# junyanz/interactive-deep-colorization

Measured on NVIDIA H100. Metric: net_forward images/sec @256x256, higher is better.
Workload: dtype f16x2-split operands, f32 accumulate (ab within 1e-3 of the f32 reference)

## Files before the change

### interactive_deep_colorization_b200/csrc/idc_api.cu

```cuda
#include <math.h>
#include <stdarg.h>
#include <stdio.h>
#include <string.h>

#include <algorithm>

#include "idc_internal.h"

using namespace idc;

struct idc_ctx : public idc::Ctx {};

namespace {

int fail(Ctx* c, int code, const char* fmt, ...) {
  char buf[512];
  va_list ap;
  va_start(ap, fmt);
  vsnprintf(buf, sizeof(buf), fmt, ap);
  va_end(ap);
  if (c) c->err = buf;
  return code;
}

// ... 545 lines not shown
                                    (size_t)nk * 2 * HW * sizeof(float), cudaMemcpyDeviceToHost, c->s_out));
      }
    } else {
      const int cap = (forked && c->click_mode && c->d_clickout) ? side_branch_cap(c) : 0;
      CUDA_TRY(c, umma_run_op(c, op, n, op.fuse_out_head ? out_ab : nullptr, (float)c->opt.tanh_scale, st, 0, cap));
    }
    mark();
  }
  const bool fused = !c->simt && !(c->flags & IDC_FLAG_KEEP_CONV10);
  if (!fused) CUDA_TRY(c, launch_out_head(c, n, out_ab, st));
  if (out_dist && !forked) {
    CUDA_TRY(c, launch_softmax529(c, n, out_dist, st));
    CUDA_TRY(c, click_tail(c, n, st));
    pdl_break(c);
  }
  if (out_rgb) {
    CUDA_TRY(c, launch_lab2rgb(c, n, c->H, c->W, L, 50.0f, out_ab, out_rgb, st, out_abq));
    c->launch_count++;
  }
  if (forked) {
    CUDA_TRY(c, cudaStreamWaitEvent(st, c->ev_join, 0));
    pdl_break(c);
  }
  mark();
  pdl_break(c);
  c->last_n = n;
  return IDC_OK;
}

int check_forward_args(Ctx* c, int n, int h, int w, const void* L, const void* ab, const void* mask, const void* glob,
                       const void* out_ab, const void* out_dist, bool resident_l_ok = false, bool hints_ok = false) {
  if (!c->weights_ready) return fail(c, IDC_ERR_STATE, "idc_forward before idc_finalize_weights");
  if (n < 1 || n > c->max_n) return fail(c, IDC_ERR_ARG, "n=%d outside [1,%d]", n, c->max_n);
  if (h != c->H || w != c->W) return fail(c, IDC_ERR_ARG, "geometry %dx%d != ctx geometry %dx%d", h, w, c->H, c->W);
  const bool hint_mode = hints_ok && !ab && !mask;
  if ((!L && !resident_l_ok) || ((!ab || !mask) && !hint_mode) || !out_ab)
    return fail(c, IDC_ERR_ARG, "null L/ab/mask/out_ab");
  if (out_dist && !c->dist) return fail(c, IDC_ERR_ARG, "out_dist requires IDC_FLAG_DIST");
  if (glob && !c->glob) return fail(c, IDC_ERR_ARG, "glob requires IDC_FLAG_GLOBAL_HINTS");
  return IDC_OK;
}

}

extern "C" {

const char* idc_version(void) { return "idc_b200 0.2 sm_90a (wgmma split-fp16 + fp32 simt engines)"; }

int idc_create(int device, int max_n, int h, int w, unsigned flags, idc_ctx** out) {
  if (!out) return IDC_ERR_ARG;
  *out = nullptr;
  if (max_n < 1 || h < 8 || w < 8 || (h % 8) || (w % 8)) return IDC_ERR_ARG;
  int ndev = 0;
  if (cudaGetDeviceCount(&ndev) != cudaSuccess || device < 0 || device >= ndev) return IDC_ERR_CUDA;
  cudaDeviceProp prop;
  if (cudaGetDeviceProperties(&prop, device) != cudaSuccess) return IDC_ERR_CUDA;
  if (prop.major != 9 || prop.minor != 0) return IDC_ERR_UNSUPPORTED;
  if (cudaSetDevice(device) != cudaSuccess) return IDC_ERR_CUDA;
  idc_ctx* c = new idc_ctx();
  c->dev = device; c->max_n = max_n; c->H = h; c->W = w; c->flags = flags;
  c->simt = flags & IDC_FLAG_ENGINE_SIMT;
  c->fast = (flags & IDC_FLAG_FAST_FP16) && !c->simt;
  c->dist = flags & IDC_FLAG_DIST;
  c->glob = flags & IDC_FLAG_GLOBAL_HINTS;
  c->caffe313 = flags & IDC_FLAG_CAFFE313;
  build_plan(c);
  int rc = alloc_workspace(c);
  if (rc != IDC_OK) {
    fprintf(stderr, "idc_create: %s\n", c->err.c_str());
    idc_destroy(c);
    return rc;
  }
  cudaStreamCreateWithFlags(&c->own_stream, cudaStreamNonBlocking);
  *out = c;
  return IDC_OK;
}

int idc_set_option(idc_ctx* c, const char* name, int value) {
  if (!c || !name) return IDC_ERR_ARG;
  struct { const char* n; int* v; } tab[] = {
      {"halo", &c->opt.halo}, {"pairs", &c->opt.pairs}, {"mt", &c->opt.mt},
      {"chunk_kb", &c->opt.chunk_kb}, {"split_k", &c->opt.split_k}, {"host_pipe", &c->opt.host_pipe},
      {"pdl", &c->opt.pdl}, {"tanh_scale", &c->opt.tanh_scale}, {"side_dist", &c->opt.side_dist},
      {"conv1_1_umma", &c->opt.conv1_1_umma}};
  for (auto& t : tab)
    if (!strcmp(t.n, name)) {
      *t.v = value;
      if (c->weights_ready && strcmp(name, "host_pipe") && strcmp(name, "tanh_scale") && strcmp(name, "side_dist") && strcmp(name, "conv1_1_umma")) {
        CUDA_TRY(c, cudaSetDevice(c->dev));
        CUDA_TRY(c, cudaDeviceSynchronize());
        int rc = plan_engines(c);
        if (rc != IDC_OK) return rc;
      }
      if (c->graph_exec) { cudaGraphExecDestroy(c->graph_exec); c->graph_exec = nullptr; }
      return IDC_OK;
    }
  return fail(c, IDC_ERR_KEY, "unknown option '%s'", name);
}

int idc_load_tensor(idc_ctx* c, const char* key, const void* data, int dtype, int ndim, const int64_t* dims) {
  if (!c || !key || !data || ndim < 0 || ndim > 8 || (ndim && !dims)) return fail(c, IDC_ERR_ARG, "bad load_tensor args");
  HostTensor t;
  size_t count = 1;
  for (int i = 0; i < ndim; ++i) {
    if (dims[i] < 0) return fail(c, IDC_ERR_ARG, "negative dim");
    t.dims.push_back(dims[i]);
    count *= (size_t)dims[i];
  }
  t.data.resize(count);
  switch (dtype) {
    case IDC_F32: memcpy(t.data.data(), data, count * sizeof(float)); break;
    case IDC_F64: for (size_t i = 0; i < count; ++i) t.data[i] = (float)((const double*)data)[i]; break;
    case IDC_I64: for (size_t i = 0; i < count; ++i) t.data[i] = (float)((const int64_t*)data)[i]; break;
    default: return fail(c, IDC_ERR_ARG, "unknown dtype %d", dtype);
  }
  c->raw[key] = std::move(t);
  c->weights_ready = false;
  return IDC_OK;
}

int idc_reserve_weights(idc_ctx* c) {
  if (!c) return IDC_ERR_ARG;
  CUDA_TRY(c, cudaSetDevice(c->dev));
  if (!c->arena) {
    c->arena_bytes = layout_arena(c, nullptr);
    CUDA_TRY(c, cudaMalloc(&c->arena, c->arena_bytes));
    layout_arena(c, c->arena);
  }
  return IDC_OK;
}

int idc_finalize_weights(idc_ctx* c) {
  if (!c) return IDC_ERR_ARG;
  int rc = idc_reserve_weights(c);
  if (rc != IDC_OK) return rc;
  std::vector<char> host(c->arena_bytes, 0);
  rc = pack_weights(c, host.data());
  if (rc != IDC_OK) return rc;
  if (c->caffe313) {
    const HostTensor* pts = find(c, "caffe.pts_in_hull");
    if (!check_dims(pts, {313, 2})) return fail(c, IDC_ERR_KEY, "missing/bad caffe.pts_in_hull [313,2]");
    CUDA_TRY(c, cudaMemcpy(c->pts313, pts->data.data(), sizeof(float) * 626, cudaMemcpyHostToDevice));
  }
  CUDA_TRY(c, cudaMemcpy(c->arena, host.data(), c->arena_bytes, cudaMemcpyHostToDevice));
  return idc_adopt_weights(c);
}

int idc_adopt_weights(idc_ctx* c) {
  if (!c || !c->arena) return fail(c, IDC_ERR_STATE, "no arena");
  CUDA_TRY(c, cudaSetDevice(c->dev));
  int rc = plan_engines(c);
  if (rc != IDC_OK) return rc;
  CUDA_TRY(c, cudaMemcpy(c->h_w11.w, c->w11, sizeof(c->h_w11.w), cudaMemcpyDeviceToHost));
  CUDA_TRY(c, cudaMemcpy(c->h_w11.b, c->b11, sizeof(c->h_w11.b), cudaMemcpyDeviceToHost));
  if (!c->simt) CUDA_TRY(c, conv1_1_umma_pack(c));
  c->raw.clear();
  c->weights_ready = true;
  if (c->graph_exec) { cudaGraphExecDestroy(c->graph_exec); c->graph_exec = nullptr; }
  return IDC_OK;
}

int idc_weights_arena(idc_ctx* c, void** dev_ptr, size_t* bytes) {
  if (!c || !dev_ptr || !bytes) return IDC_ERR_ARG;
  if (!c->arena) return fail(c, IDC_ERR_STATE, "arena not allocated");
  *dev_ptr = c->arena; *bytes = c->arena_bytes;
  return IDC_OK;
}
// ... 703 lines not shown
```

### interactive_deep_colorization_b200/csrc/idc_internal.h

```cpp
#pragma once
#include <cuda.h>
#include <cuda_fp16.h>
#include <cuda_runtime.h>
#include <stdint.h>

#include <map>
#include <string>
#include <vector>

#include "../../include/idc_b200.h"

namespace idc {

constexpr int kMaxTaps = 34;
constexpr int kMaxSrc = 6;
constexpr int kMaxCls = 4;

enum Act { ACT_NONE = 0, ACT_RELU = 1, ACT_LEAKY02 = 2 };

constexpr int kActScaleLog2 = 6;
constexpr float kActScale = 64.0f;
constexpr float kActInvScale = 1.0f / 64.0f;

struct Tap {
  int src;
  int ky, kx;
  int ty, tx;
};

struct ActBuf {
  std::string name;
  int H = 0, W = 0, C = 0;
  void* p0 = nullptr;
  void* p1 = nullptr;
};

struct Epilogue {
  float* bias = nullptr;
  float* scale = nullptr;
  float* shift = nullptr;
  int act = ACT_NONE;
  bool has_bn = false;
  bool gadd = false;
};

struct SrcDesc {
  int buf = -1;
  int s = 1;
  int cin = 0;
};

enum OpKind { OP_CONV = 0, OP_UP = 1, OP_CLASS = 2, OP_HYPER = 3 };

struct ConvOp {
  std::string name;
  int kind = OP_CONV;
  std::string wkey[kMaxSrc];
  bool src_deconv[kMaxSrc] = {false, false, false, false, false, false};
  int src_k[kMaxSrc] = {3, 3, 3, 3, 3, 3};
  std::string bnkey;
  int nsrc = 1;
  SrcDesc src[kMaxSrc];
  int ncls = 1;
  int ntaps = 0;
  Tap taps[kMaxCls][kMaxTaps];
  int Hl = 0, Wl = 0;
  int out_buf = -1;
  int os = 1;
  int cout = 0, cout_pad = 0;
  int K = 0;
  Epilogue epi;
  bool fuse_out_head = false;
  bool out_f32 = false;
  float* out_f32_ptr = nullptr;
  float* w_simt = nullptr;
  __half* w_hi = nullptr;
  __half* w_lo = nullptr;
  int bn_tile = 0, hbox = 0, wbox = 0;
  void* umma_plan = nullptr;
  double flops_per_image = 0;
};

struct Conv11Weights {
  float w[36 * 64];
  float b[64];
};

struct Options {
  int halo = 1;
  int pairs = 0;
  int mt = -1;
  int chunk_kb = -1;
  int split_k = -1;
  int host_pipe = 1;
  int pdl = 1;
  int conv1_1_umma = 1;
  int side_dist = 1;
  int tanh_scale = 110;
};

struct HostTensor {
  std::vector<float> data;
  std::vector<int64_t> dims;
};

struct Ctx {
  int dev = 0;
  int max_n = 0, H = 0, W = 0;
  unsigned flags = 0;
  Options opt;
  bool simt = false, fast = false, dist = false, glob = false;
  std::map<std::string, HostTensor> raw;
  std::vector<ActBuf> bufs;
  std::map<std::string, int> buf_index;
  std::vector<ConvOp> ops;
  char* arena = nullptr;
  size_t arena_bytes = 0;
  bool weights_ready = false;
  float* w11 = nullptr;
  float* b11 = nullptr;
  Conv11Weights h_w11;
  uint8_t* w11_umma = nullptr;
  float* wout = nullptr;
  float* bout = nullptr;
  float* gw[4] = {nullptr, nullptr, nullptr, nullptr};
  float* gb[4] = {nullptr, nullptr, nullptr, nullptr};
  float* gscale[4] = {nullptr, nullptr, nullptr, nullptr};
  float* gshift[4] = {nullptr, nullptr, nullptr, nullptr};
  float* gvec = nullptr;
  float* gtmp = nullptr;
  float* logits = nullptr;
  float* logits313 = nullptr;
  bool caffe313 = false;
  float* pts313 = nullptr;
  float* splitk_ws = nullptr; size_t splitk_ws_floats = 0;
  int* splitk_counters = nullptr; int splitk_max_tiles = 0;
  bool dbg_graph_timing = false;
  cudaEvent_t dbg_ev[2] = {nullptr, nullptr};
  float dbg_graph_ms = 0.f;
  int* d_err = nullptr;
  int* h_err = nullptr;
  float* h_in = nullptr;  float* d_in = nullptr;   size_t in_floats = 0;
  float* h_out = nullptr; float* d_out = nullptr;  size_t out_floats = 0;
  uint8_t* h_rgb = nullptr; uint8_t* d_rgb = nullptr;
  char* h_small = nullptr; char* d_small = nullptr;
  double* h_abq = nullptr; double* d_abq = nullptr;
  cudaStream_t own_stream = nullptr;
  cudaStream_t s_in = nullptr, s_out = nullptr;
  cudaStream_t s_side = nullptr;
  cudaEvent_t ev_fork = nullptr, ev_join = nullptr;
  cudaStream_t s_click = nullptr;
  cudaEvent_t ev_click[2] = {nullptr, nullptr};
  int image_n = 0;
  char* h_hints = nullptr; char* d_hints = nullptr;
  int graph_captures = 0;
  cudaEvent_t ev_in[8] = {}, ev_out[8] = {};
  cudaGraphExec_t graph_exec = nullptr;
  const void* graph_ptrs[8] = {nullptr};
  float graph_maskcent = 0.f;
  int launch_count = 0;
  int graph_launches = 0;
  bool chain = false;
  bool gadd_active = false;
  int last_n = 0;
  double* d_reccs = nullptr;
  bool dist_resident = false;
  int dist_valid_n = 0;
  bool click_mode = false;
  int* h_click = nullptr; int* d_click = nullptr;
  char* d_clickout = nullptr; char* h_clickout = nullptr;
  bool click_served = false;
  bool profiling = false;
  std::vector<std::vector<cudaEvent_t>> prof_runs;
  std::vector<cudaEvent_t> prof_pool;
  std::string err;
};
// ... 67 lines not shown
```

### interactive_deep_colorization_b200/csrc/idc_umma.cu

```cuda
#include <stdio.h>
#include <stdlib.h>

#include "idc_internal.h"

namespace idc {

constexpr int kBM = 128;
constexpr int kBK = 64;
constexpr int kThreads = 384;
constexpr int kProdRegs = 40;
constexpr int kMathRegs = 232;
constexpr int kMathThreads = 256;

struct UmmaParams {
  const CUtensorMap* amaps;
  const int4* kblk;
  int nkb, ncls;
  int chunk_kb;
  int split_k;
  float* ws;
  int* counters;
  int n_img, tiles_y, tiles_x, n_tiles_n, total_tiles;
  int hbox, wbox, wshift;
  int Hl, Wl, cout_pad;
  const float* bias;
  const float* scale;
  const float* shift;
  const float* gadd;
  int gadd_ld;
  float gadd_mult;
  int act;
  __half* out_hi;
  __half* out_lo;
  int Hout, Wout, Cout, os;
  float* out_f32;
  int out_ld;
  const float* wout;
  const float* bout;
  float* out_ab;
  float out_mult;
  int* err;
  int n_amaps;
  int max_ctas;
  int img0;
};

__device__ __forceinline__ uint32_t smem_u32(const void* p) { return (uint32_t)__cvta_generic_to_shared(p); }

__device__ __forceinline__ void mbar_init(uint32_t bar, uint32_t count) {
  asm volatile("mbarrier.init.shared::cta.b64 [%0], %1;" ::"r"(bar), "r"(count));
}
__device__ __forceinline__ void mbar_expect_tx(uint32_t bar, uint32_t bytes) {
  asm volatile("mbarrier.arrive.expect_tx.shared::cta.b64 _, [%0], %1;" ::"r"(bar), "r"(bytes) : "memory");
}
__device__ __forceinline__ void mbar_arrive(uint32_t bar) {
  asm volatile("mbarrier.arrive.shared::cta.b64 _, [%0];" ::"r"(bar) : "memory");
}
__device__ __forceinline__ uint32_t mbar_try_wait(uint32_t bar, uint32_t parity) {
  uint32_t ok;
  asm volatile(
      "{\n\t.reg .pred p;\n\t"
      "mbarrier.try_wait.parity.shared::cta.b64 p, [%1], %2;\n\t"
      "selp.u32 %0, 1, 0, p;\n\t}"
      : "=r"(ok)
      : "r"(bar), "r"(parity)
      : "memory");
  return ok;
}
__device__ __noinline__ void mbar_timeout(int* err, int code) {
  if (err) {
    atomicExch(err, code);
    __threadfence_system();
  }
  __trap();
}
__device__ __forceinline__ void mbar_wait(uint32_t bar, uint32_t parity, int* err, int code) {
  if (mbar_try_wait(bar, parity)) return;
  const long long t0 = clock64();
  while (!mbar_try_wait(bar, parity)) {
    if (clock64() - t0 > 6000000000LL) mbar_timeout(err, code);
  }
}

__device__ __forceinline__ bool elect_one() {
// ... 65 lines not shown
template <int N>
__device__ __forceinline__ void wgmma_wait() { asm volatile("wgmma.wait_group.sync.aligned %0;" ::"n"(N) : "memory"); }
template <int R>
__device__ __forceinline__ void wgmma_reg_fence(float (&d)[R]) {
#pragma unroll
  for (int i = 0; i < R; ++i) asm volatile("" : "+f"(d[i])::"memory");
}

__device__ __forceinline__ void wgmma_n64(float (&d)[32], uint64_t adesc, uint64_t bdesc, uint32_t accumulate) {
  asm volatile(
      "{\n\t.reg .pred p;\n\t"
      "setp.ne.b32 p, %34, 0;\n\t"
      "wgmma.mma_async.sync.aligned.m64n64k16.f32.f16.f16 "
      "{%0, %1, %2, %3, %4, %5, %6, %7, %8, %9, %10, %11, %12, %13, %14, %15, %16, %17, %18, %19, %20, %21, %22, %23, %24, %25, %26, %27, %28, %29, %30, %31}, "
      "%32, %33, p, 1, 1, 0, 0;\n\t}"
      : "+f"(d[0]), "+f"(d[1]), "+f"(d[2]), "+f"(d[3]), "+f"(d[4]), "+f"(d[5]), "+f"(d[6]), "+f"(d[7]), "+f"(d[8]), "+f"(d[9]), "+f"(d[10]), "+f"(d[11]), "+f"(d[12]), "+f"(d[13]), "+f"(d[14]), "+f"(d[15]), "+f"(d[16]), "+f"(d[17]), "+f"(d[18]), "+f"(d[19]), "+f"(d[20]), "+f"(d[21]), "+f"(d[22]), "+f"(d[23]), "+f"(d[24]), "+f"(d[25]), "+f"(d[26]), "+f"(d[27]), "+f"(d[28]), "+f"(d[29]), "+f"(d[30]), "+f"(d[31])
      : "l"(adesc), "l"(bdesc), "r"(accumulate));
}

__device__ __forceinline__ void wgmma_n128(float (&d)[64], uint64_t adesc, uint64_t bdesc, uint32_t accumulate) {
  asm volatile(
      "{\n\t.reg .pred p;\n\t"
      "setp.ne.b32 p, %66, 0;\n\t"
      "wgmma.mma_async.sync.aligned.m64n128k16.f32.f16.f16 "
      "{%0, %1, %2, %3, %4, %5, %6, %7, %8, %9, %10, %11, %12, %13, %14, %15, %16, %17, %18, %19, %20, %21, %22, %23, %24, %25, %26, %27, %28, %29, %30, %31, %32, %33, %34, %35, %36, %37, %38, %39, %40, %41, %42, %43, %44, %45, %46, %47, %48, %49, %50, %51, %52, %53, %54, %55, %56, %57, %58, %59, %60, %61, %62, %63}, "
      "%64, %65, p, 1, 1, 0, 0;\n\t}"
      : "+f"(d[0]), "+f"(d[1]), "+f"(d[2]), "+f"(d[3]), "+f"(d[4]), "+f"(d[5]), "+f"(d[6]), "+f"(d[7]), "+f"(d[8]), "+f"(d[9]), "+f"(d[10]), "+f"(d[11]), "+f"(d[12]), "+f"(d[13]), "+f"(d[14]), "+f"(d[15]), "+f"(d[16]), "+f"(d[17]), "+f"(d[18]), "+f"(d[19]), "+f"(d[20]), "+f"(d[21]), "+f"(d[22]), "+f"(d[23]), "+f"(d[24]), "+f"(d[25]), "+f"(d[26]), "+f"(d[27]), "+f"(d[28]), "+f"(d[29]), "+f"(d[30]), "+f"(d[31]), "+f"(d[32]), "+f"(d[33]), "+f"(d[34]), "+f"(d[35]), "+f"(d[36]), "+f"(d[37]), "+f"(d[38]), "+f"(d[39]), "+f"(d[40]), "+f"(d[41]), "+f"(d[42]), "+f"(d[43]), "+f"(d[44]), "+f"(d[45]), "+f"(d[46]), "+f"(d[47]), "+f"(d[48]), "+f"(d[49]), "+f"(d[50]), "+f"(d[51]), "+f"(d[52]), "+f"(d[53]), "+f"(d[54]), "+f"(d[55]), "+f"(d[56]), "+f"(d[57]), "+f"(d[58]), "+f"(d[59]), "+f"(d[60]), "+f"(d[61]), "+f"(d[62]), "+f"(d[63])
      : "l"(adesc), "l"(bdesc), "r"(accumulate));
}

template <int BN>
__device__ __forceinline__ void wgmma_bn(float (&d)[BN / 2], uint64_t adesc, uint64_t bdesc, uint32_t accumulate) {
  if constexpr (BN == 128) wgmma_n128(d, adesc, bdesc, accumulate);
  else wgmma_n64(d, adesc, bdesc, accumulate);
}

__device__ __forceinline__ uint64_t make_sw128_desc(uint32_t smem_addr, uint32_t sbo = 1024u) {
  uint64_t d = 0;
  d |= (uint64_t)((smem_addr >> 4) & 0x3FFFu);
  d |= (uint64_t)1 << 16;
  d |= (uint64_t)(sbo >> 4) << 32;
  d |= (uint64_t)1 << 62;
  return d;
}

__device__ __forceinline__ uint32_t pack_f16x2_sat(float a, float b) {
  uint32_t r;
  asm("cvt.rn.satfinite.f16x2.f32 %0, %1, %2;" : "=r"(r) : "f"(b), "f"(a));
  return r;
}
__device__ __forceinline__ uint32_t lo_f16x2(float a, float b, uint32_t hw) {
  const float2 hf = __half22float2(*reinterpret_cast<const __half2*>(&hw));
  return pack_f16x2_sat(a - hf.x, b - hf.y);
}

__device__ __forceinline__ void split_h(float v, __half& hi, __half& lo) {
  v = fminf(fmaxf(v, -65504.f), 65504.f);
  hi = __float2half_rn(v);
  lo = __float2half_rn(v - __half2float(hi));
}

__device__ __forceinline__ int frag_col(int i, int lane) { return 8 * (i >> 2) + 2 * (lane & 3) + (i & 1); }

constexpr int kHaloW = 10, kHaloH = 18;
constexpr int kHaloPlane = (kHaloW * kHaloH * 128 + 1023) / 1024 * 1024;


template <int BN, int MT, int CG, bool SPLIT, bool HALO>
struct SmemPlan {
  static constexpr int kABytes = MT * kBM * kBK * 2;
  static constexpr int kAStage = HALO ? 0 : kABytes;
  static constexpr int kBBytes = BN * kBK * 2;
  static constexpr int kStageBytes = (SPLIT ? 2 : 1) * (kAStage + kBBytes);
  static constexpr int kHaloSlot = (SPLIT ? 2 : 1) * kHaloPlane;
  static constexpr int kHaloBytes = HALO ? 2 * kHaloSlot : 0;
  static constexpr int kOutRow = 64 * 2 + 16;
  static constexpr int kOutWarp = 16 * kOutRow;
  static constexpr int kOutStage = 8 * kOutWarp;
  static constexpr int kTail = 3 * BN * 4 + 272 * 4 + 256;
  static constexpr int kBudget = 232448 - 1024 - kTail - kOutStage - kHaloBytes;
  static constexpr int kStages = kBudget / kStageBytes >= 4 ? 4 : kBudget / kStageBytes;
  static constexpr int kTotal = kStages * kStageBytes + kHaloBytes + kOutStage + kTail + 1024;
  static_assert(kStages >= 2, "need at least a double-buffered operand ring");
  static_assert(MT * BN <= 128, "register budget: chunk + tile accumulators of MT*BN columns per math thread pair");
  static_assert(!HALO || MT == 1, "halo tiles are single 16x8-pixel M-tiles");
  static_assert(CG == 1 || CG == 2, "clusters of one or two CTAs");
};

template <int BN, int MT, int CG, bool SPLIT, bool HALO>
__global__ void __launch_bounds__(kThreads, 1)
umma_conv_kernel(const __grid_constant__ CUtensorMap bmap_hi, const __grid_constant__ CUtensorMap bmap_lo,
                 const __grid_constant__ UmmaParams p) {
  using SP = SmemPlan<BN, MT, CG, SPLIT, HALO>;
  constexpr int STAGES = SP::kStages;
  constexpr int R = BN / 2;
  constexpr bool PAIR = CG == 2;
  extern __shared__ uint8_t smem_raw[];
  uint8_t* smem = reinterpret_cast<uint8_t*>((reinterpret_cast<uintptr_t>(smem_raw) + 1023) & ~uintptr_t(1023));
  uint8_t* s_halo = smem + STAGES * SP::kStageBytes;
  uint8_t* s_out = s_halo + SP::kHaloBytes;
  float* s_bias = reinterpret_cast<float*>(s_out + SP::kOutStage);
  float* s_scale = s_bias + BN;
  float* s_shift = s_scale + BN;
  float* s_head = s_shift + BN;
  uint64_t* full_bar = reinterpret_cast<uint64_t*>(s_head + 272);
  uint64_t* empty_bar = full_bar + 4;
  uint64_t* afull_bar = full_bar + 8;
  uint64_t* aempty_bar = full_bar + 10;

  const int warp = threadIdx.x >> 5, lane = threadIdx.x & 31;
  const uint32_t cta_rank = PAIR ? cluster_ctarank() : 0u;

  if (p.wout) {
    for (int i = threadIdx.x; i < 256; i += kThreads) s_head[i] = p.wout[i];
    if (threadIdx.x < 2) s_head[256 + threadIdx.x] = p.bout[threadIdx.x];
  }
  if (threadIdx.x == 32) {
    prefetch_tmap(&bmap_hi);
    if (SPLIT) prefetch_tmap(&bmap_lo);
    for (int i = 0; i < p.n_amaps; ++i) prefetch_tmap(p.amaps + i);
  }
  if (threadIdx.x == 0) {
    for (int s = 0; s < STAGES; ++s) {
      mbar_init(smem_u32(&full_bar[s]), 1);
      mbar_init(smem_u32(&empty_bar[s]), 8 * CG);
    }
    if (HALO)
      for (int a = 0; a < 2; ++a) {
        mbar_init(smem_u32(&afull_bar[a]), 1);
        mbar_init(smem_u32(&aempty_bar[a]), 8);
      }
    asm volatile("fence.mbarrier_init.release.cluster;" ::: "memory");
  }
  if (PAIR) cluster_sync_all(); else __syncthreads();
  pdl_launch_dependents();
  pdl_wait();

  const int tiles_per_img = p.tiles_y * p.tiles_x;
  const int S = p.split_k;
  const int n_items = p.total_tiles * S;
  const int w0 = blockIdx.x / CG, wstep = gridDim.x / CG;

  if (warp < 4) {
    asm volatile("setmaxnreg.dec.sync.aligned.u32 %0;" ::"n"(kProdRegs));
    if (warp == 0) {
      int stage = 0;
      uint32_t phase = 0;
      uint32_t hcount = 0;
      for (int w = w0; w < n_items; w += wstep) {
        const int tile = w / S, ks = w - tile * S;
        const int kbeg = (ks * p.nkb) / S, kend = ((ks + 1) * p.nkb) / S;
        int r = tile;
        const int nt = r % p.n_tiles_n;
        r /= p.n_tiles_n;
        const int cls = r % p.ncls;
        r /= p.ncls;
        if (PAIR) r = 2 * r + (int)cta_rank;
        const int img_rel = r / tiles_per_img;
        r -= img_rel * tiles_per_img;
        const int img = p.img0 + img_rel;
        const int y0 = (r / p.tiles_x) * (p.hbox * MT), x0 = (r % p.tiles_x) * p.wbox;
        const int brow = cls * p.cout_pad + nt * BN + (int)cta_rank * (BN / CG);
        const int4* kb = p.kblk + cls * p.nkb;
        for (int k = kbeg; k < kend; ++k) {
          if (HALO && k % 9 == 0) {
            const uint32_t slot = hcount & 1, hphase = (hcount >> 1) & 1;
            ++hcount;
            mbar_wait(smem_u32(&aempty_bar[slot]), hphase ^ 1, p.err, 6);
            if (elect_one()) {
              const uint32_t fa = smem_u32(&afull_bar[slot]);
              const uint32_t sh = smem_u32(s_halo + slot * SP::kHaloSlot);
              const int c0 = (k / 9) * kBK;
              mbar_expect_tx(fa, (SPLIT ? 2 : 1) * kHaloW * kHaloH * 128);
              tma_load_4d(sh, p.amaps, fa, c0, x0 - 1, y0 - 1, img);
              if (SPLIT) tma_load_4d(sh + kHaloPlane, p.amaps + 1, fa, c0, x0 - 1, y0 - 1, img);
            }
            __syncwarp();
          }
          mbar_wait(smem_u32(&empty_bar[stage]), phase ^ 1, p.err, 1);
          if (elect_one()) {
            const uint32_t fb = smem_u32(&full_bar[stage]);
            const int4 e = __ldg(kb + k);
            const uint32_t sa = smem_u32(smem + stage * SP::kStageBytes);
            const uint32_t sb = sa + (SPLIT ? 2 : 1) * SP::kAStage + cta_rank * (BN / CG) * 128;
            const int kcol = HALO ? e.y : k * kBK;
            mbar_expect_tx(fb, SP::kStageBytes);
            if (!HALO) {
              const CUtensorMap* am = p.amaps + e.x;
              tma_load_4d(sa, am, fb, e.y, x0 + e.w, y0 + e.z, img);
              if (SPLIT) tma_load_4d(sa + SP::kABytes, am + 1, fb, e.y, x0 + e.w, y0 + e.z, img);
            }
            if (PAIR) {
              tma_load_2d_mc(sb, &bmap_hi, fb, kcol, brow);
              if (SPLIT) tma_load_2d_mc(sb + SP::kBBytes, &bmap_lo, fb, kcol, brow);
            } else {
              tma_load_2d(sb, &bmap_hi, fb, kcol, brow);
              if (SPLIT) tma_load_2d(sb + SP::kBBytes, &bmap_lo, fb, kcol, brow);
            }
          }
          __syncwarp();
          if (++stage == STAGES) { stage = 0; phase ^= 1; }
        }
      }
    }
  } else {
    asm volatile("setmaxnreg.inc.sync.aligned.u32 %0;" ::"n"(kMathRegs));
    const int et = threadIdx.x - 128;
    const int wg = et >> 7;
    const int wi = (et >> 5) & 3;
    const uint32_t wbuf = smem_u32(s_out) + (uint32_t)(et >> 5) * SP::kOutWarp;
    auto release = [&](uint64_t* bar) {
      __syncwarp();
      if (lane == 0) {
        mbar_arrive(smem_u32(bar));
        if (PAIR) mbar_arrive_remote(smem_u32(bar), cta_rank ^ 1u);
      }
    };
    int stage = 0;
    uint32_t phase = 0;
    uint32_t hcount = 0;
    int staged_key = -1;
    for (int w = w0; w < n_items; w += wstep) {
      const int tile = w / S, ks = w - tile * S;
      const int kbeg = (ks * p.nkb) / S, kend = ((ks + 1) * p.nkb) / S;
      int r = tile;
      const int nt = r % p.n_tiles_n;
      r /= p.n_tiles_n;
      const int cls = r % p.ncls;
      r /= p.ncls;
      if (PAIR) r = 2 * r + (int)cta_rank;
      const int img_rel = r / tiles_per_img;
      r -= img_rel * tiles_per_img;
      const int img = p.img0 + img_rel;
      const int ty0 = (r / p.tiles_x) * (p.hbox * MT), tx0 = (r % p.tiles_x) * p.wbox;
      const int n0 = nt * BN;
      const int vkey = p.gadd ? (img * p.n_tiles_n + nt) : nt;
      if (vkey != staged_key) {
        asm volatile("bar.sync 1, 256;" ::: "memory");
        for (int i = et; i < BN; i += kMathThreads) {
          s_bias[i] = p.bias[n0 + i];
          s_scale[i] = p.scale[n0 + i];
          const int gi = img < p.n_img ? img : p.n_img - 1;
          s_shift[i] = p.shift[n0 + i] + (p.gadd ? p.gadd[(size_t)gi * p.gadd_ld + n0 + i] * p.gadd_mult : 0.f);
        }
        asm volatile("bar.sync 1, 256;" ::: "memory");
        staged_key = vkey;
      }

      float acc[MT][R];
#pragma unroll
      for (int m = 0; m < MT; ++m)
#pragma unroll
        for (int j = 0; j < R; ++j) acc[m][j] = 0.f;
      for (int k0 = kbeg; k0 < kend; k0 += p.chunk_kb) {
        const int k1 = (k0 + p.chunk_kb < kend) ? k0 + p.chunk_kb : kend;
        float part[MT][R];
#pragma unroll
        for (int m = 0; m < MT; ++m)
#pragma unroll
          for (int j = 0; j < R; ++j) part[m][j] = 0.f;
        int prev = -1;
        for (int k = k0; k < k1; ++k) {
          uint32_t hslot = 0;
          if (HALO) {
            if (k % 9 == 0) {
              mbar_wait(smem_u32(&afull_bar[hcount & 1]), (hcount >> 1) & 1, p.err, 7);
              ++hcount;
            }
            hslot = (hcount - 1) & 1;
          }
          mbar_wait(smem_u32(&full_bar[stage]), phase, p.err, 3);
          const uint32_t st0 = smem_u32(smem + stage * SP::kStageBytes);
          const uint32_t sb = st0 + (SPLIT ? 2 : 1) * SP::kAStage;
          const uint64_t b_hi = make_sw128_desc(sb), b_lo = make_sw128_desc(sb + SP::kBBytes);
          uint32_t ha = 0;
          if (HALO) {
            const int4 e = __ldg(p.kblk + k);
            ha = smem_u32(s_halo + hslot * SP::kHaloSlot) + (uint32_t)((e.z + wg * 8) * kHaloW + e.w) * 128u;
          }
          wgmma_fence();
#pragma unroll
          for (int m = 0; m < MT; ++m) {
            const uint32_t sa = st0 + (uint32_t)(wg * MT + m) * (64 * 128);
            const uint64_t a_hi = HALO ? make_sw128_desc(ha, kHaloW * 128) : make_sw128_desc(sa);
            const uint64_t a_lo = HALO ? make_sw128_desc(ha + kHaloPlane, kHaloW * 128) : make_sw128_desc(sa + SP::kABytes);
            uint32_t first = (k == k0) ? 0u : 1u;
            if (SPLIT) {
#pragma unroll
              for (int kk = 0; kk < kBK / 16; ++kk) {
                const uint64_t adv = (uint64_t)(kk * 2);
                wgmma_bn<BN>(part[m], a_lo + adv, b_hi + adv, first);
                wgmma_bn<BN>(part[m], a_hi + adv, b_lo + adv, 1u);
                first = 1u;
              }
            }
#pragma unroll
            for (int kk = 0; kk < kBK / 16; ++kk) {
              const uint64_t adv = (uint64_t)(kk * 2);
              wgmma_bn<BN>(part[m], a_hi + adv, b_hi + adv, first);
              first = 1u;
            }
          }
          wgmma_commit();
          if (HALO && k % 9 == 8) {
            wgmma_wait<0>();
            __syncwarp();
            if (lane == 0) mbar_arrive(smem_u32(&aempty_bar[hslot]));
          }
          if (prev >= 0) {
            wgmma_wait<1>();
            release(&empty_bar[prev]);
          }
          prev = stage;
          if (++stage == STAGES) { stage = 0; phase ^= 1; }
        }
        wgmma_wait<0>();
#pragma unroll
        for (int m = 0; m < MT; ++m) wgmma_reg_fence(part[m]);
        release(&empty_bar[prev]);
#pragma unroll
        for (int m = 0; m < MT; ++m)
#pragma unroll
          for (int j = 0; j < R; ++j) acc[m][j] += part[m][j];
      }

      if (S > 1) {
        float* wp = p.ws + (size_t)w * R * kMathThreads + et;
#pragma unroll
        for (int i = 0; i < R; ++i)
          if ((i >> 4) % S != ks) __stcg(wp + (size_t)i * kMathThreads, acc[0][i]);
        __threadfence();
        asm volatile("bar.sync 1, 256;" ::: "memory");
        if (et == 0) {
          int* cnt = p.counters + 2 * tile;
          atomicAdd(cnt, 1);
          const long long t0 = clock64();
          int seen;
          do {
            asm volatile("ld.acquire.gpu.global.s32 %0, [%1];" : "=r"(seen) : "l"(cnt) : "memory");
            if (seen < S && clock64() - t0 > 6000000000LL) mbar_timeout(p.err, 5);
          } while (seen < S);
        }
        asm volatile("bar.sync 1, 256;" ::: "memory");
        for (int q = 0; q < S; ++q) {
          if (q == ks) continue;
          const float* rp = p.ws + (size_t)(tile * S + q) * R * kMathThreads + et;
#pragma unroll
          for (int i = 0; i < R; ++i)
            if ((i >> 4) % S == ks) acc[0][i] += __ldcg(rp + (size_t)i * kMathThreads);
        }
      }

      const float neg_slope = p.act == ACT_RELU ? 0.f : (p.act == ACT_LEAKY02 ? 0.2f : 1.f);
#pragma unroll
      for (int m = 0; m < MT; ++m) {
        const int blk = (wg * MT + m) * 64;
#pragma unroll
        for (int i = 0; i < R; ++i) {
          const int c = frag_col(i, lane);
          const float t = acc[m][i] + s_bias[c];
          acc[m][i] = fmaf(fmaxf(t, neg_slope * t), s_scale[c], s_shift[c]);
        }
        int ry[2], rx[2];
        bool ok[2];
#pragma unroll
        for (int h = 0; h < 2; ++h) {
          const int rr = blk + wi * 16 + (lane >> 2) + 8 * h;
          ry[h] = ty0 + (rr >> p.wshift);
          rx[h] = tx0 + (rr & (p.wbox - 1));
          ok[h] = ry[h] < p.Hl && rx[h] < p.Wl && img < p.n_img;
        }
        if (p.wout) {
          float h0[2] = {0.f, 0.f}, h1[2] = {0.f, 0.f};
#pragma unroll
          for (int i = 0; i < R; ++i) {
            const int c = frag_col(i, lane), h = (i >> 1) & 1;
            h0[h] = fmaf(acc[m][i], s_head[c], h0[h]);
            h1[h] = fmaf(acc[m][i], s_head[128 + c], h1[h]);
          }
#pragma unroll
          for (int h = 0; h < 2; ++h) {
#pragma unroll
            for (int o = 1; o <= 2; o <<= 1) {
              h0[h] += __shfl_xor_sync(0xffffffffu, h0[h], o);
              h1[h] += __shfl_xor_sync(0xffffffffu, h1[h], o);
            }
            if ((lane & 3) == 0 && ok[h]) {
              const size_t HW = (size_t)p.Hl * p.Wl;
              const size_t o = (size_t)img * 2 * HW + (size_t)ry[h] * p.Wl + rx[h];
              p.out_ab[o] = tanhf(h0[h] + s_head[256]) * p.out_mult;
              p.out_ab[o + HW] = tanhf(h1[h] + s_head[257]) * p.out_mult;
            }
          }
        } else if (p.out_f32) {
#pragma unroll
          for (int i = 0; i < R; i += 2) {
            const int h = (i >> 1) & 1;
            if ((S > 1 && (i >> 4) % S != ks) || !ok[h]) continue;
            float* o = p.out_f32 + ((size_t)(img * p.Hl + ry[h]) * p.Wl + rx[h]) * p.out_ld + n0 + frag_col(i, lane);
            *reinterpret_cast<float2*>(o) = make_float2(acc[m][i], acc[m][i + 1]);
          }
        } else {
          __half* prow[4];
          const int rl0 = lane >> 3, ch = lane & 7;
#pragma unroll
          for (int it = 0; it < 4; ++it) {
            const int rr = blk + wi * 16 + rl0 + 4 * it;
// ... 268 lines not shown
  CUtensorMap bmap_hi, bmap_lo;
  UmmaParams prm{};
  int num_sms = 132;
  int dev = 0;
  int mt = 1;
  int cg = 1;
  int split_k = 1;
  bool halo = false;
  size_t ws_floats = 0;
  int ws_tiles = 0;
};

struct ViewKey {
  int src, s, qy, qx;
  bool operator==(const ViewKey& o) const { return src == o.src && s == o.s && qy == o.qy && qx == o.qx; }
};

static int floordiv2(int v) { return v >= 0 ? v / 2 : -((-v + 1) / 2); }

template <int BN, int MT, int CG, bool SPLIT, bool HALO = false>
static cudaError_t launch_inst(const UmmaPlan& pl, const UmmaParams& prm, cudaStream_t st, bool pdl) {
  using SP = SmemPlan<BN, MT, CG, SPLIT, HALO>;
  static unsigned long long attr_devs = 0;
  if (pl.dev >= 64 || !(attr_devs & (1ull << pl.dev))) {
    cudaError_t e = cudaFuncSetAttribute(umma_conv_kernel<BN, MT, CG, SPLIT, HALO>, cudaFuncAttributeMaxDynamicSharedMemorySize,
                                         SP::kTotal);
    if (e != cudaSuccess) return e;
    if (pl.dev < 64) attr_devs |= 1ull << pl.dev;
  }
  const long items = (long)prm.total_tiles * prm.split_k;
  int grid = items * CG < pl.num_sms ? (int)items * CG : (pl.num_sms / CG) * CG;
  if (prm.max_ctas > 0 && grid > prm.max_ctas) grid = prm.max_ctas;
  cudaLaunchConfig_t cfg{};
  cfg.gridDim = dim3(grid);
  cfg.blockDim = dim3(kThreads);
  cfg.dynamicSmemBytes = SP::kTotal;
  cfg.stream = st;
  cudaLaunchAttribute at[2];
  int na = 0;
  if (CG > 1) {
    at[na].id = cudaLaunchAttributeClusterDimension;
    at[na].val.clusterDim.x = CG; at[na].val.clusterDim.y = 1; at[na].val.clusterDim.z = 1;
    ++na;
  }
  if (pdl) {
    at[na].id = cudaLaunchAttributeProgrammaticStreamSerialization;
    at[na].val.programmaticStreamSerializationAllowed = 1;
    ++na;
  }
  cfg.attrs = at;
  cfg.numAttrs = na;
  return cudaLaunchKernelEx(&cfg, umma_conv_kernel<BN, MT, CG, SPLIT, HALO>, pl.bmap_hi, pl.bmap_lo, prm);
}

int umma_plan_op(Ctx* c, ConvOp& op) {
  PFN_encodeTiled enc = get_encode();
  if (!enc) { c->err = "cuTensorMapEncodeTiled entry point not available"; return IDC_ERR_CUDA; }
  umma_free_op(op);
  UmmaPlan* pl = new UmmaPlan();
  op.umma_plan = pl;
  cudaDeviceProp prop;
  cudaGetDeviceProperties(&prop, c->dev);
  pl->num_sms = prop.multiProcessorCount;
  pl->dev = c->dev;
  op.bn_tile = (op.cout_pad % 128 == 0) ? 128 : 64;
  if (op.cout_pad % op.bn_tile) { c->err = "cout not tileable: " + op.name; return IDC_ERR_ARG; }
  if (op.fuse_out_head && op.cout_pad != 128) { c->err = "fused model_out needs 128 columns: " + op.name; return IDC_ERR_ARG; }
  int best = 1 << 30;
  for (int wb = 128; wb >= 8; wb >>= 1) {
    const int hb = kBM / wb;
    const int t = ceil_div(op.Wl, wb) * ceil_div(op.Hl, hb);
    if (t < best) { best = t; op.wbox = wb; op.hbox = hb; }
  }
  {
    const int mode = c->opt.halo;
    bool ok = mode >= 1 && !c->fast && op.ncls == 1 && op.ntaps == 9;
    unsigned seen = 0;
    for (int t = 0; ok && t < op.ntaps; ++t) {
      const Tap& tp = op.taps[0][t];
      if (tp.src != op.taps[0][0].src || op.src[tp.src].s != 1 || tp.ty < -1 || tp.ty > 1 || tp.tx < -1 || tp.tx > 1) ok = false;
      else seen |= 1u << ((tp.ty + 1) * 3 + tp.tx + 1);
    }
    if (ok && (seen != 0x1FFu || op.src[op.taps[0][0].src].cin % kBK)) ok = false;
    if (ok && !(op.bn_tile == 128 || (mode >= 3 && op.bn_tile == 64))) ok = false;
    if (ok) {
      const long T = (long)c->max_n * ceil_div(op.Hl, 16) * ceil_div(op.Wl, 8) * (op.cout_pad / op.bn_tile);
      if (T < 2L * pl->num_sms && mode < 3) ok = false;
    }
    pl->halo = ok;
    if (ok) { op.wbox = 8; op.hbox = 16; }
  }
  pl->mt = 1;
  if (op.bn_tile == 64 && !pl->halo && !op.fuse_out_head) {
    const long tiles2 = (long)op.ncls * c->max_n * ceil_div(op.Hl, 2 * op.hbox) * ceil_div(op.Wl, op.wbox) *
                        (op.cout_pad / op.bn_tile);
    if (tiles2 >= 2L * pl->num_sms) pl->mt = 2;
  }
  {
    const int v = c->opt.mt;
    if (!pl->halo && v == 1) pl->mt = 1;
    if (!pl->halo && v == 2 && !op.fuse_out_head) { pl->mt = 2; op.bn_tile = 64; }
  }
  pl->cg = 1;
  {
    const long tiles_mt = (long)op.ncls * c->max_n * ceil_div(op.Hl, op.hbox * pl->mt) * ceil_div(op.Wl, op.wbox) *
                          (op.cout_pad / op.bn_tile);
    const int mode = c->opt.pairs;
    if (!c->fast && (mode >= 2 || (mode == 1 && tiles_mt >= 2L * pl->num_sms))) pl->cg = 2;
  }
  const int nkb = op.K / kBK;
  {
    const int ty = ceil_div(op.Hl, op.hbox * pl->mt), tx = ceil_div(op.Wl, op.wbox), ntn = op.cout_pad / op.bn_tile;
    const long T = (long)op.ncls * c->max_n * ty * tx * ntn;
    const bool eligible = nkb >= 8 && !op.fuse_out_head && pl->mt == 1 && pl->cg == 1 && !pl->halo;
    int S = 1;
    if (T * 2 <= pl->num_sms && eligible) {
      S = (int)(pl->num_sms / T);
      if (S > nkb / 4) S = nkb / 4;
      if (S > op.bn_tile / 32) S = op.bn_tile / 32;
      if (S < 1) S = 1;
    }
    {
      const int v = c->opt.split_k;
      if (eligible && v >= 1 && v <= nkb && v <= op.bn_tile / 32 && T * v <= pl->num_sms) S = v;
    }
    pl->split_k = S;
    pl->ws_tiles = (int)T;
    pl->ws_floats = S > 1 ? (size_t)T * S * kBM * op.bn_tile : 0;
    if (pl->ws_floats > c->splitk_ws_floats) c->splitk_ws_floats = pl->ws_floats;
    if (S > 1 && pl->ws_tiles > c->splitk_max_tiles) c->splitk_max_tiles = pl->ws_tiles;
  }
  std::vector<ViewKey> views;
  std::vector<int4> kblk((size_t)op.ncls * nkb);
  if (pl->halo) {
    const int src = op.taps[0][0].src, groups = op.src[src].cin / kBK;
    views.push_back(ViewKey{src, 1, 0, 0});
    for (int i = 0; i < nkb; ++i) {
      const int g = i / 9, t = i % 9;
      kblk[i] = make_int4(0, (t * groups + g) * kBK, op.taps[0][t].ty + 1, op.taps[0][t].tx + 1);
    }
  }
  for (int cls = 0; cls < op.ncls && !pl->halo; ++cls) {
    int kb = 0;
    for (int t = 0; t < op.ntaps; ++t) {
      const Tap& tp = op.taps[cls][t];
      const int s = op.src[tp.src].s;
      ViewKey vk{tp.src, s, 0, 0};
      int dy = tp.ty, dx = tp.tx;
      if (s == 2) {
        vk.qy = ((tp.ty % 2) + 2) % 2; vk.qx = ((tp.tx % 2) + 2) % 2;
        dy = floordiv2(tp.ty); dx = floordiv2(tp.tx);
      }
      int vi = -1;
      for (size_t i = 0; i < views.size(); ++i)
        if (views[i] == vk) vi = (int)i;
      if (vi < 0) { views.push_back(vk); vi = (int)views.size() - 1; }
      const int cin = op.src[tp.src].cin;
      if (cin % kBK) { c->err = "cin not a multiple of 64: " + op.name; return IDC_ERR_ARG; }
      for (int c0 = 0; c0 < cin; c0 += kBK) kblk[(size_t)cls * nkb + kb++] = make_int4(vi * 2, c0, dy, dx);
    }
    if (kb != nkb) { c->err = "k-block count mismatch: " + op.name; return IDC_ERR_ARG; }
  }
  std::vector<CUtensorMap> amaps(views.size() * 2);
  for (size_t i = 0; i < views.size(); ++i) {
    const ViewKey& vk = views[i];
    const ActBuf& b = c->bufs[op.src[vk.src].buf];
    const int Hv = (b.H - vk.qy + vk.s - 1) / vk.s, Wv = (b.W - vk.qx + vk.s - 1) / vk.s;
// ... 11 lines not shown
                       CU_TENSOR_MAP_INTERLEAVE_NONE, CU_TENSOR_MAP_SWIZZLE_128B, CU_TENSOR_MAP_L2_PROMOTION_L2_128B,
                       CU_TENSOR_MAP_FLOAT_OOB_FILL_NONE);
      if (r != CUDA_SUCCESS) {
        char msg[256];
        snprintf(msg, sizeof(msg), "cuTensorMapEncodeTiled(A) failed (%d) for op %s view %zu", (int)r, op.name.c_str(), i);
        c->err = msg;
        return IDC_ERR_CUDA;
      }
    }
  }
  for (int part = 0; part < 2; ++part) {
    cuuint64_t dims[2] = {(cuuint64_t)op.K, (cuuint64_t)op.ncls * op.cout_pad};
    cuuint64_t strides[1] = {(cuuint64_t)op.K * 2};
    cuuint32_t box[2] = {(cuuint32_t)kBK, (cuuint32_t)(op.bn_tile / pl->cg)};
    cuuint32_t estr[2] = {1, 1};
    CUresult r = enc(part == 0 ? &pl->bmap_hi : &pl->bmap_lo, CU_TENSOR_MAP_DATA_TYPE_FLOAT16, 2,
                     part == 0 ? (void*)op.w_hi : (void*)op.w_lo, dims, strides, box, estr,
                     CU_TENSOR_MAP_INTERLEAVE_NONE, CU_TENSOR_MAP_SWIZZLE_128B, CU_TENSOR_MAP_L2_PROMOTION_L2_256B,
                     CU_TENSOR_MAP_FLOAT_OOB_FILL_NONE);
    if (r != CUDA_SUCCESS) {
      char msg[256];
      snprintf(msg, sizeof(msg), "cuTensorMapEncodeTiled(B) failed (%d) for op %s", (int)r, op.name.c_str());
      c->err = msg;
      return IDC_ERR_CUDA;
    }
  }
  if (cudaMalloc(&pl->d_amaps, amaps.size() * sizeof(CUtensorMap)) != cudaSuccess ||
      cudaMalloc(&pl->d_kblk, kblk.size() * sizeof(int4)) != cudaSuccess) {
    c->err = "cudaMalloc failed in umma_plan_op";
    return IDC_ERR_CUDA;
  }
  cudaMemcpy(pl->d_amaps, amaps.data(), amaps.size() * sizeof(CUtensorMap), cudaMemcpyHostToDevice);
  cudaMemcpy(pl->d_kblk, kblk.data(), kblk.size() * sizeof(int4), cudaMemcpyHostToDevice);

  UmmaParams& q = pl->prm;
  q.amaps = pl->d_amaps; q.n_amaps = (int)amaps.size(); q.kblk = pl->d_kblk; q.nkb = nkb; q.ncls = op.ncls;
  {
    const int natural = (op.cout_pad % 256 == 0) ? 256 : (op.cout_pad % 192 == 0) ? 192 : (op.cout_pad % 128 == 0) ? 128 : 64;
    int g = c->fast ? 4 : (natural <= 128 ? 2 : 1);
    if (c->opt.chunk_kb >= 1) g = c->opt.chunk_kb;
    q.chunk_kb = g;
  }
  q.tiles_y = ceil_div(op.Hl, op.hbox * pl->mt); q.tiles_x = ceil_div(op.Wl, op.wbox);
  q.n_tiles_n = op.cout_pad / op.bn_tile;
  q.hbox = op.hbox; q.wbox = op.wbox;
  q.wshift = 0;
  while ((1 << q.wshift) < op.wbox) q.wshift++;
  q.Hl = op.Hl; q.Wl = op.Wl; q.cout_pad = op.cout_pad;
  q.bias = op.epi.bias; q.scale = op.epi.scale; q.shift = op.epi.shift;
  q.gadd = nullptr; q.gadd_ld = 512; q.gadd_mult = kActScale;
  q.act = op.epi.act;
  if (op.out_f32) {
    q.out_f32 = op.out_f32_ptr; q.out_ld = op.cout_pad;
  } else if (op.out_buf >= 0) {
    const ActBuf& ob = c->bufs[op.out_buf];
    q.out_hi = (__half*)ob.p0; q.out_lo = (__half*)ob.p1;
    q.Hout = ob.H; q.Wout = ob.W; q.Cout = ob.C; q.os = op.os;
  }
  if (op.fuse_out_head) { q.wout = c->wout; q.bout = c->bout; }
  q.err = c->d_err;
  q.img0 = 0;
  return IDC_OK;
}

void umma_free_op(ConvOp& op) {
  UmmaPlan* pl = static_cast<UmmaPlan*>(op.umma_plan);
  if (!pl) return;
  if (pl->d_amaps) cudaFree(pl->d_amaps);
  if (pl->d_kblk) cudaFree(pl->d_kblk);
  delete pl;
  op.umma_plan = nullptr;
}

bool umma_op_uses_split_k(const ConvOp& op) {
  const UmmaPlan* pl = static_cast<const UmmaPlan*>(op.umma_plan);
  return pl && pl->split_k > 1;
}

cudaError_t umma_run_op(Ctx* c, ConvOp& op, int n, float* out_ab_fused, float out_mult, cudaStream_t st, int img0,
                        int max_ctas) {
  UmmaPlan* pl = static_cast<UmmaPlan*>(op.umma_plan);
  if (!pl) return cudaErrorInvalidValue;
  UmmaParams prm = pl->prm;
  prm.max_ctas = (max_ctas > 0 && pl->split_k == 1) ? (max_ctas / pl->cg) * pl->cg : 0;
  prm.img0 = img0;
  prm.n_img = img0 + n;
  if (img0 && pl->split_k > 1) return cudaErrorInvalidValue;
  const int m_tiles = n * prm.tiles_y * prm.tiles_x;
  prm.total_tiles = op.ncls * (pl->cg == 2 ? (m_tiles + 1) / 2 : m_tiles) * prm.n_tiles_n;
  prm.gadd = (op.epi.gadd && c->gadd_active) ? c->gvec : nullptr;
  prm.out_ab = out_ab_fused;
  prm.split_k = pl->split_k;
  prm.ws = c->splitk_ws;
  prm.counters = c->splitk_counters;
  if (pl->split_k > 1 && (!prm.ws || !prm.counters)) return cudaErrorInvalidValue;
  prm.out_mult = out_mult;
  if (op.fuse_out_head && !out_ab_fused) return cudaErrorInvalidValue;
  c->launch_count++;
  const bool pdl = pdl_take(c);
  const bool split = !c->fast;
  if (pl->halo) {
    if (!split) return cudaErrorInvalidValue;
    switch (op.bn_tile * 10 + pl->cg) {
      case 641: return launch_inst<64, 1, 1, true, true>(*pl, prm, st, pdl);
      case 642: return launch_inst<64, 1, 2, true, true>(*pl, prm, st, pdl);
      case 1281: return launch_inst<128, 1, 1, true, true>(*pl, prm, st, pdl);
      case 1282: return launch_inst<128, 1, 2, true, true>(*pl, prm, st, pdl);
      default: return cudaErrorInvalidValue;
    }
  }
#define IDC_LAUNCH(BN_, MT_, CG_) \
  return split ? launch_inst<BN_, MT_, CG_, true>(*pl, prm, st, pdl) : launch_inst<BN_, MT_, CG_, false>(*pl, prm, st, pdl)
  switch (op.bn_tile * 100 + pl->mt * 10 + pl->cg) {
    case 6411: IDC_LAUNCH(64, 1, 1);
    case 6421: IDC_LAUNCH(64, 2, 1);
    case 12811: IDC_LAUNCH(128, 1, 1);
    case 6412: return launch_inst<64, 1, 2, true>(*pl, prm, st, pdl);
    case 6422: return launch_inst<64, 2, 2, true>(*pl, prm, st, pdl);
    case 12812: return launch_inst<128, 1, 2, true>(*pl, prm, st, pdl);
    default: break;
  }
#undef IDC_LAUNCH
  return cudaErrorInvalidValue;
}

}
```

Measured before the change: 1032.

## Overlap WGMMA chunks across K-chunk boundaries with double-buffered partial accumulators

Restructures the math-warp K loop so successive split-precision chunks use alternating partial accumulators. The fold of one chunk into the tile accumulator and the release of its stage now happen while the next chunk's WGMMAs are in flight, rather than draining with wait<0> at every chunk end and every halo-slot boundary. It also lets halo mode apply to 64-wide N tiles without requiring mode 3, and adds a max_ctas option to cap the persistent grid. This costs extra accumulator registers and more complex barrier and halo-slot release ordering.

```diff
diff --git a/interactive_deep_colorization_b200/csrc/idc_api.cu b/interactive_deep_colorization_b200/csrc/idc_api.cu
--- a/interactive_deep_colorization_b200/csrc/idc_api.cu
+++ b/interactive_deep_colorization_b200/csrc/idc_api.cu
@@ -651,7 +651,7 @@
       {"halo", &c->opt.halo}, {"pairs", &c->opt.pairs}, {"mt", &c->opt.mt},
       {"chunk_kb", &c->opt.chunk_kb}, {"split_k", &c->opt.split_k}, {"host_pipe", &c->opt.host_pipe},
       {"pdl", &c->opt.pdl}, {"tanh_scale", &c->opt.tanh_scale}, {"side_dist", &c->opt.side_dist},
-      {"conv1_1_umma", &c->opt.conv1_1_umma}};
+      {"conv1_1_umma", &c->opt.conv1_1_umma}, {"max_ctas", &c->opt.max_ctas}};
   for (auto& t : tab)
     if (!strcmp(t.n, name)) {
       *t.v = value;
diff --git a/interactive_deep_colorization_b200/csrc/idc_internal.h b/interactive_deep_colorization_b200/csrc/idc_internal.h
--- a/interactive_deep_colorization_b200/csrc/idc_internal.h
+++ b/interactive_deep_colorization_b200/csrc/idc_internal.h
@@ -92,6 +92,7 @@
   int mt = -1;
   int chunk_kb = -1;
   int split_k = -1;
+  int max_ctas = 0;
   int host_pipe = 1;
   int pdl = 1;
   int conv1_1_umma = 1;
diff --git a/interactive_deep_colorization_b200/csrc/idc_umma.cu b/interactive_deep_colorization_b200/csrc/idc_umma.cu
--- a/interactive_deep_colorization_b200/csrc/idc_umma.cu
+++ b/interactive_deep_colorization_b200/csrc/idc_umma.cu
@@ -1,5 +1,7 @@
 #include <stdio.h>
 #include <stdlib.h>
+
+#include <type_traits>
 
 #include "idc_internal.h"
 
@@ -231,7 +233,8 @@
   static constexpr int kStages = kBudget / kStageBytes >= 4 ? 4 : kBudget / kStageBytes;
   static constexpr int kTotal = kStages * kStageBytes + kHaloBytes + kOutStage + kTail + 1024;
   static_assert(kStages >= 2, "need at least a double-buffered operand ring");
-  static_assert(MT * BN <= 128, "register budget: chunk + tile accumulators of MT*BN columns per math thread pair");
+  static_assert(MT * BN <= 128, "register budget: the tile accumulator and two chunk accumulators of MT*BN/2 registers "
+                                "each (3 x 64 of a math thread's 232 at MT*BN = 128)");
   static_assert(!HALO || MT == 1, "halo tiles are single 16x8-pixel M-tiles");
   static_assert(CG == 1 || CG == 2, "clusters of one or two CTAs");
 };
@@ -369,9 +372,89 @@
     uint32_t phase = 0;
     uint32_t hcount = 0;
     int staged_key = -1;
+    const bool pipe_chunks = HALO || p.chunk_kb > 1;
+    int k = 0, kend = 0;
+    int prev = -1;
+    int hfree = -1;
+    float acc[MT][R];
+    float part[2][MT][R];
+    auto retire_prev = [&]() {
+      release(&empty_bar[prev]);
+      if (HALO && hfree >= 0 && lane == 0) mbar_arrive(smem_u32(&aempty_bar[hfree]));
+    };
+    auto fold = [&](float (&pt)[MT][R]) {
+#pragma unroll
+      for (int m = 0; m < MT; ++m) wgmma_reg_fence(pt[m]);
+#pragma unroll
+      for (int m = 0; m < MT; ++m)
+#pragma unroll
+        for (int j = 0; j < R; ++j) acc[m][j] += pt[m][j];
+    };
+    auto chunk_step = [&](auto par) -> bool {
+      constexpr int P = decltype(par)::value;
+      const int kc = k, k1 = (k + p.chunk_kb < kend) ? k + p.chunk_kb : kend;
+      for (; k < k1; ++k) {
+        uint32_t hslot = 0;
+        if (HALO) {
+          if (k % 9 == 0) {
+            mbar_wait(smem_u32(&afull_bar[hcount & 1]), (hcount >> 1) & 1, p.err, 7);
+            ++hcount;
+          }
+          hslot = (hcount - 1) & 1;
+        }
+        mbar_wait(smem_u32(&full_bar[stage]), phase, p.err, 3);
+        const uint32_t st0 = smem_u32(smem + stage * SP::kStageBytes);
+        const uint32_t sb = st0 + (SPLIT ? 2 : 1) * SP::kAStage;
+        const uint64_t b_hi = make_sw128_desc(sb), b_lo = make_sw128_desc(sb + SP::kBBytes);
+        uint32_t ha = 0;
+        if (HALO) {
+          const int4 e = __ldg(p.kblk + k);
+          ha = smem_u32(s_halo + hslot * SP::kHaloSlot) + (uint32_t)((e.z + wg * 8) * kHaloW + e.w) * 128u;
+        }
+        wgmma_fence();
+#pragma unroll
+        for (int m = 0; m < MT; ++m) {
+          const uint32_t sa = st0 + (uint32_t)(wg * MT + m) * (64 * 128);
+          const uint64_t a_hi = HALO ? make_sw128_desc(ha, kHaloW * 128) : make_sw128_desc(sa);
+          const uint64_t a_lo = HALO ? make_sw128_desc(ha + kHaloPlane, kHaloW * 128) : make_sw128_desc(sa + SP::kABytes);
+          uint32_t first = (k == kc) ? 0u : 1u;
+          if (SPLIT) {
+#pragma unroll
+            for (int kk = 0; kk < kBK / 16; ++kk) {
+              const uint64_t adv = (uint64_t)(kk * 2);
+              wgmma_bn<BN>(part[P][m], a_lo + adv, b_hi + adv, first);
+              wgmma_bn<BN>(part[P][m], a_hi + adv, b_lo + adv, 1u);
+              first = 1u;
+            }
+          }
+#pragma unroll
+          for (int kk = 0; kk < kBK / 16; ++kk) {
+            const uint64_t adv = (uint64_t)(kk * 2);
+            wgmma_bn<BN>(part[P][m], a_hi + adv, b_hi + adv, first);
+            first = 1u;
+          }
+        }
+        wgmma_commit();
+        if (prev >= 0) {
+          wgmma_wait<1>();
+          retire_prev();
+          if (k == kc) fold(part[P ^ 1]);
+        }
+        prev = stage;
+        hfree = (HALO && k % 9 == 8) ? (int)hslot : -1;
+        if (++stage == STAGES) { stage = 0; phase ^= 1; }
+      }
+      if (k < kend && pipe_chunks) return false;
+      wgmma_wait<0>();
+      retire_prev();
+      fold(part[P]);
+      prev = -1;
+      return HALO ? true : k == kend;
+    };
     for (int w = w0; w < n_items; w += wstep) {
       const int tile = w / S, ks = w - tile * S;
-      const int kbeg = (ks * p.nkb) / S, kend = ((ks + 1) * p.nkb) / S;
+      k = (ks * p.nkb) / S;
+      kend = ((ks + 1) * p.nkb) / S;
       int r = tile;
       const int nt = r % p.n_tiles_n;
       r /= p.n_tiles_n;
@@ -396,82 +479,12 @@
         staged_key = vkey;
       }
 
-      float acc[MT][R];
 #pragma unroll
       for (int m = 0; m < MT; ++m)
 #pragma unroll
-        for (int j = 0; j < R; ++j) acc[m][j] = 0.f;
-      for (int k0 = kbeg; k0 < kend; k0 += p.chunk_kb) {
-        const int k1 = (k0 + p.chunk_kb < kend) ? k0 + p.chunk_kb : kend;
-        float part[MT][R];
-#pragma unroll
-        for (int m = 0; m < MT; ++m)
-#pragma unroll
-          for (int j = 0; j < R; ++j) part[m][j] = 0.f;
-        int prev = -1;
-        for (int k = k0; k < k1; ++k) {
-          uint32_t hslot = 0;
-          if (HALO) {
-            if (k % 9 == 0) {
-              mbar_wait(smem_u32(&afull_bar[hcount & 1]), (hcount >> 1) & 1, p.err, 7);
-              ++hcount;
-            }
-            hslot = (hcount - 1) & 1;
-          }
-          mbar_wait(smem_u32(&full_bar[stage]), phase, p.err, 3);
-          const uint32_t st0 = smem_u32(smem + stage * SP::kStageBytes);
-          const uint32_t sb = st0 + (SPLIT ? 2 : 1) * SP::kAStage;
-          const uint64_t b_hi = make_sw128_desc(sb), b_lo = make_sw128_desc(sb + SP::kBBytes);
-          uint32_t ha = 0;
-          if (HALO) {
-            const int4 e = __ldg(p.kblk + k);
-            ha = smem_u32(s_halo + hslot * SP::kHaloSlot) + (uint32_t)((e.z + wg * 8) * kHaloW + e.w) * 128u;
-          }
-          wgmma_fence();
-#pragma unroll
-          for (int m = 0; m < MT; ++m) {
-            const uint32_t sa = st0 + (uint32_t)(wg * MT + m) * (64 * 128);
-            const uint64_t a_hi = HALO ? make_sw128_desc(ha, kHaloW * 128) : make_sw128_desc(sa);
-            const uint64_t a_lo = HALO ? make_sw128_desc(ha + kHaloPlane, kHaloW * 128) : make_sw128_desc(sa + SP::kABytes);
-            uint32_t first = (k == k0) ? 0u : 1u;
-            if (SPLIT) {
-#pragma unroll
-              for (int kk = 0; kk < kBK / 16; ++kk) {
-                const uint64_t adv = (uint64_t)(kk * 2);
-                wgmma_bn<BN>(part[m], a_lo + adv, b_hi + adv, first);
-                wgmma_bn<BN>(part[m], a_hi + adv, b_lo + adv, 1u);
-                first = 1u;
-              }
-            }
-#pragma unroll
-            for (int kk = 0; kk < kBK / 16; ++kk) {
-              const uint64_t adv = (uint64_t)(kk * 2);
-              wgmma_bn<BN>(part[m], a_hi + adv, b_hi + adv, first);
-              first = 1u;
-            }
-          }
-          wgmma_commit();
-          if (HALO && k % 9 == 8) {
-            wgmma_wait<0>();
-            __syncwarp();
-            if (lane == 0) mbar_arrive(smem_u32(&aempty_bar[hslot]));
-          }
-          if (prev >= 0) {
-            wgmma_wait<1>();
-            release(&empty_bar[prev]);
-          }
-          prev = stage;
-          if (++stage == STAGES) { stage = 0; phase ^= 1; }
-        }
-        wgmma_wait<0>();
-#pragma unroll
-        for (int m = 0; m < MT; ++m) wgmma_reg_fence(part[m]);
-        release(&empty_bar[prev]);
-#pragma unroll
-        for (int m = 0; m < MT; ++m)
-#pragma unroll
-          for (int j = 0; j < R; ++j) acc[m][j] += part[m][j];
-      }
+        for (int j = 0; j < R; ++j) acc[m][j] = part[0][m][j] = part[1][m][j] = 0.f;
+      for (int par = 0;; par ^= 1)
+        if (par ? chunk_step(std::integral_constant<int, 1>{}) : chunk_step(std::integral_constant<int, 0>{})) break;
 
       if (S > 1) {
         float* wp = p.ws + (size_t)w * R * kMathThreads + et;
@@ -906,7 +919,7 @@
       else seen |= 1u << ((tp.ty + 1) * 3 + tp.tx + 1);
     }
     if (ok && (seen != 0x1FFu || op.src[op.taps[0][0].src].cin % kBK)) ok = false;
-    if (ok && !(op.bn_tile == 128 || (mode >= 3 && op.bn_tile == 64))) ok = false;
+
     if (ok) {
       const long T = (long)c->max_n * ceil_div(op.Hl, 16) * ceil_div(op.Wl, 8) * (op.cout_pad / op.bn_tile);
       if (T < 2L * pl->num_sms && mode < 3) ok = false;
@@ -1084,6 +1097,8 @@
   UmmaPlan* pl = static_cast<UmmaPlan*>(op.umma_plan);
   if (!pl) return cudaErrorInvalidValue;
   UmmaParams prm = pl->prm;
+  if (c->opt.max_ctas > 0 && (max_ctas <= 0 || c->opt.max_ctas < max_ctas)) max_ctas = c->opt.max_ctas;
+  if (max_ctas > 0 && max_ctas < pl->cg) max_ctas = pl->cg;
   prm.max_ctas = (max_ctas > 0 && pl->split_k == 1) ? (max_ctas / pl->cg) * pl->cg : 0;
   prm.img0 = img0;
   prm.n_img = img0 + n;
```

Result: faster. 1052, median of 6 (+2.0%).
